# shanedirksen/gnn-plasma-flux

Hardware: AMD Instinct MI355X
Metric: hybrid rollout timesteps/sec (batched ICs) at 1/2/4/8 MI355X (higher is better)
Workload: dtype f32

## Files before the change

gnn-plasma-flux_amd/csrc/chain_bf16.hip:

```cpp
#include "chain_common.h"

namespace hf {
namespace {

using namespace chain;

typedef __bf16 b8 __attribute__((ext_vector_type(8)));
typedef __bf16 b2 __attribute__((ext_vector_type(2)));
typedef float f2 __attribute__((ext_vector_type(2)));
typedef unsigned u4 __attribute__((ext_vector_type(4)));

__device__ __forceinline__ unsigned pk_bf16(float a, float b) {
  return __builtin_bit_cast(unsigned, __builtin_convertvector(f2{a, b}, b2));
}
__device__ __forceinline__ unsigned pk_relu_bf16(float a, float b) { return pk_bf16(relu(a), relu(b)); }
__device__ __forceinline__ f4 mma(const u4 &a, const u4 &b, f4 c) {
  return __builtin_amdgcn_mfma_f32_16x16x32_bf16(__builtin_bit_cast(b8, a), __builtin_bit_cast(b8, b), c, 0, 0, 0);
}

template <int NM, int NV, int ND = 4>
__device__ __forceinline__ void interleave() {
  __builtin_amdgcn_sched_group_barrier(0x100, ND, 0);
#pragma unroll
  for (int i = 0; i < NM; ++i) {
    __builtin_amdgcn_sched_group_barrier(0x008, 1, 0);
    __builtin_amdgcn_sched_group_barrier(0x002, NV, 0);
  }
  __builtin_amdgcn_sched_barrier(0);
}

template <int NW, int UPC, int WMT = 4, bool PF = false, int SLOTS = (UPC == 4 ? 3 : 4), int WG = 1, int DMAU = 0,
          bool XCH = false, bool LDR = false>
struct CoreBF16 {
  static_assert(!XCH || (UPC == 4 && !PF && WMT == 4), "super-window core: 16 KiB chunks, 64-cell waves");
  static constexpr int kNW = NW;
  static constexpr int kWGPerCU = WG;
  static constexpr int kUPC = UPC;
  static constexpr int kSlots = SLOTS;
  static constexpr int kAhead = 2;
  static constexpr int kWinMT = WMT;
  static constexpr int kParkMT = WMT;
  static constexpr int kChunkFloats = 1024 * UPC;
  static constexpr int kKB = kH / 32;
  static constexpr int kStreamOffset = XCH ? kBF16StreamTail : 0;
  static constexpr int kParkFloats = 3 * kParkMT * 64 * 4;
  static constexpr int kSeamF4 = XCH ? 2 * NW * 2 * 4 * 2 : 0;
  static constexpr int kDmaUnit = DMAU;
  using R_t = Ring<kChunkFloats, NW, kSlots, 2, (DMAU >= 0), LDR>;
  static constexpr int pos(int U) { return XCH ? (U + 2) & 3 : U % UPC; }

  template <int MT>
  struct Acts {
    u4 h[MT][kKB];
  };
  template <int MT>
  struct Pair {
    f4 a[MT][2], g[MT][2];
  };

  struct Seam {
    f4 *pubw;
    f4 *rdl;
    f4 *rdr;
    int par;
    static __device__ __forceinline__ int slot(int w, int side) { return (w * 2 + side) * 8; }
    static __device__ __forceinline__ int lane_id() {
      int l;
      asm volatile("v_mbcnt_lo_u32_b32 %0, -1, 0\n\tv_mbcnt_hi_u32_b32 %0, -1, %0" : "=v"(l));
      return l;
    }
  };
  template <int MT>
  static __device__ __forceinline__ void publish(const Seam &sm, const Pair<MT> &P) {
#if defined(HF_DIAG_NOSEAM) || defined(HF_DIAG_NOPUB)
    return;
#endif
    if constexpr (XCH) {
      const int l = Seam::lane_id(), j = l & 15;
      f4 *p = sm.pubw + sm.par * (NW * 16) + ((l >> 4) << 1);
      if (j == 0) {
        p[0] = P.g[1][0];
        p[1] = P.g[1][1];
      }
      if (j == 15) {
        p[8] = P.g[MT - 2][0];
        p[9] = P.g[MT - 2][1];
      }
    }
  }
  static __device__ __forceinline__ void seam_read(const Seam &sm, int t, f4 &L, f4 &R) {
#if defined(HF_DIAG_NOSEAM) || defined(HF_DIAG_NORD)
    L = R = f4{0.f, 0.f, 0.f, 0.f};
    return;
#endif
    const int l = Seam::lane_id(), o = sm.par * (NW * 16) + ((l >> 4) << 1) + t;
    L = sm.rdl[o];
    R = sm.rdr[o];
  }

  struct Feed {
    const float *slot;
    u4 cur[4];
  };
  static __device__ __forceinline__ void load_unit(Feed &F, int u, int lane) {
#pragma unroll
    for (int i = 0; i < 4; ++i) F.cur[i] = __builtin_bit_cast(u4, ldf4(F.slot + ((4 * u + i) * 64 + lane) * 4));
  }
  static __device__ __forceinline__ void begin(R_t &R, Feed &F) {
    F.slot = R.next();
    if constexpr (XCH) R.issue_pending();
    if constexpr (PF) load_unit(F, 0, R.lane);
  }
  template <int U>
  static __device__ __forceinline__ void take(R_t &R, Feed &F, u4 (&w)[4]) {
    if constexpr (PF) {
#pragma unroll
      for (int i = 0; i < 4; ++i) w[i] = F.cur[i];
      if constexpr (U == kDmaUnit) R.issue_pending();
      if constexpr (U == UPC - 1) F.slot = R.next();
      load_unit(F, (U + 1) % UPC, R.lane);
    } else {
#ifdef HF_DIAG_NODS
#pragma unroll
      for (int i = 0; i < 4; ++i) w[i] = u4{(unsigned)R.lane, (unsigned)(4 * U + i), 0x3f803f80u, (unsigned)R.lane};
#else
#pragma unroll
      for (int i = 0; i < 4; ++i) w[i] = __builtin_bit_cast(u4, ldf4(F.slot + ((4 * U + i) * 64 + R.lane) * 4));
#endif
      if constexpr (U == kDmaUnit) R.issue_pending();
      if constexpr (U == UPC - 1) F.slot = R.next();
    }
  }

  static __device__ __forceinline__ float *park_at(float *park, int kb, int mt, int lane) {
    return park + ((kb * kParkMT + mt) * 64 + lane) * 4;
  }

  template <int MT, int KB>
  static __device__ __forceinline__ void unit_mfma(const u4 (&w)[4], const Acts<MT> &X, Pair<MT> &P) {
#pragma unroll
    for (int t = 0; t < 2; ++t)
#pragma unroll
      for (int mt = 0; mt < MT; ++mt) {
        P.a[mt][t] = mma(w[2 * t], X.h[mt][KB], P.a[mt][t]);
        P.g[mt][t] = mma(w[2 * t + 1], X.h[mt][KB], P.g[mt][t]);
      }
  }
  template <int MT, int KB>
  static __device__ __forceinline__ void unit(R_t &R, Feed &F, const Acts<MT> &X, Pair<MT> &P) {
    u4 w[4];
    take<pos(KB)>(R, F, w);
    unit_mfma<MT, KB>(w, X, P);
  }

  template <int MT>
  static __device__ __forceinline__ void init(const float *bias, int q, int g4, Pair<MT> &P) {
#pragma unroll
    for (int t = 0; t < 2; ++t) {
      const f4 b = ldf4(bias + 16 * (2 * q + t) + g4);
#pragma unroll
      for (int mt = 0; mt < MT; ++mt) {
        P.a[mt][t] = b;
        P.g[mt][t] = f4{0.f, 0.f, 0.f, 0.f};
      }
    }
  }

  template <int MT, int K, int PART = 0>
  static __device__ __forceinline__ void piece(Pair<MT> &P, u4 (&nh)[MT], const f4 &L = f4{}, const f4 &R = f4{}) {
    constexpr int t = K >> 1, r0 = 2 * (K & 1);
#ifdef HF_DIAG_NOPIECE
#pragma unroll
    for (int mt = 0; mt < MT; ++mt)
      if (PART == 0 || (PART == 1) == (mt > 0 && mt < MT - 1)) nh[mt][K] = pk_bf16(P.a[mt][t][r0], P.g[mt][t][r0 + 1]);
    return;
#endif
    if constexpr (PART == 0) {
      float z[2][MT];
#pragma unroll
      for (int rr = 0; rr < 2; ++rr) {
        float v[MT], sm[MT];
#pragma unroll
        for (int mt = 0; mt < MT; ++mt) v[mt] = P.g[mt][t][r0 + rr];
        nb_sum<MT>(v, sm);
#pragma unroll
        for (int mt = 0; mt < MT; ++mt) z[rr][mt] = __fadd_rn(P.a[mt][t][r0 + rr], sm[mt]);
      }
#pragma unroll
      for (int mt = 0; mt < MT; ++mt) nh[mt][K] = pk_relu_bf16(z[0][mt], z[1][mt]);
    } else if constexpr (PART == 1) {
#pragma unroll
      for (int mt = 1; mt < MT - 1; ++mt) {
        float z[2];
#pragma unroll
        for (int rr = 0; rr < 2; ++rr) {
          const int r = r0 + rr;
          z[rr] = __fadd_rn(P.a[mt][t][r], __fadd_rn(P.g[mt - 1][t][r], P.g[mt + 1][t][r]));
        }
        nh[mt][K] = pk_relu_bf16(z[0], z[1]);
      }
    } else {
      float z0[2], z1[2];
#pragma unroll
      for (int rr = 0; rr < 2; ++rr) {
        const int r = r0 + rr;
        float sl = __fadd_rn(L[r], P.g[1][t][r]);
        asm("v_add_f32_dpp %0, %1, %2 row_shr:1 row_mask:0xf bank_mask:0xf"
            : "+v"(sl)
            : "v"(P.g[MT - 1][t][r]), "v"(P.g[1][t][r]));
        z0[rr] = __fadd_rn(P.a[0][t][r], sl);
        float sr = __fadd_rn(R[r], P.g[MT - 2][t][r]);
        asm("v_add_f32_dpp %0, %1, %2 row_shl:1 row_mask:0xf bank_mask:0xf"
            : "+v"(sr)
            : "v"(P.g[0][t][r]), "v"(P.g[MT - 2][t][r]));
        z1[rr] = __fadd_rn(P.a[MT - 1][t][r], sr);
      }
      nh[0][K] = pk_relu_bf16(z0[0], z0[1]);
      nh[MT - 1][K] = pk_relu_bf16(z1[0], z1[1]);
    }
  }

  template <int MT>
  static __device__ __forceinline__ void pair_with_prev(R_t &R, Feed &F, const Acts<MT> &X, const float *bias, int q,
                                                        int g4, Pair<MT> &acc, Pair<MT> &prev, float *park,
                                                        int lane, Seam &sm) {
    init<MT>(bias, q, g4, acc);
    u4 nh[MT];
    if constexpr (XCH) {
      unit<MT, 0>(R, F, X, acc);
      piece<MT, 0, 1>(prev, nh);
      piece<MT, 1, 1>(prev, nh);
      interleave<4 * MT, 2>();
      publish<MT>(sm, prev);
      unit<MT, 1>(R, F, X, acc);
      f4 L0, R0;
      seam_read(sm, 0, L0, R0);
      piece<MT, 2, 1>(prev, nh);
      piece<MT, 0, 2>(prev, nh, L0, R0);
      interleave<4 * MT, 2, 2>();
      unit<MT, 2>(R, F, X, acc);
      f4 L1, R1;
      seam_read(sm, 1, L1, R1);
      piece<MT, 3, 1>(prev, nh);
      piece<MT, 1, 2>(prev, nh, L0, R0);
      interleave<4 * MT, 2, 6>();
      unit<MT, 3>(R, F, X, acc);
      piece<MT, 2, 2>(prev, nh, L1, R1);
      piece<MT, 3, 2>(prev, nh, L1, R1);
      sm.par ^= 1;
    } else {
      unit<MT, 0>(R, F, X, acc);
      piece<MT, 0>(prev, nh);
      interleave<4 * MT, 2>();
      unit<MT, 1>(R, F, X, acc);
      piece<MT, 1>(prev, nh);
      interleave<4 * MT, 2>();
      unit<MT, 2>(R, F, X, acc);
      piece<MT, 2>(prev, nh);
      interleave<4 * MT, 2>();
      unit<MT, 3>(R, F, X, acc);
      piece<MT, 3>(prev, nh);
    }
#pragma unroll
    for (int mt = 0; mt < MT; ++mt) *reinterpret_cast<u4 *>(park_at(park, q - 1, mt, lane)) = nh[mt];
    interleave<4 * MT, 2>();
  }

  template <int MT>
  static __device__ __forceinline__ void pair0_after(R_t &R, Feed &F, Acts<MT> &X, const float *bias, int g4,
                                                     Pair<MT> &acc, Pair<MT> &pend, float *park, int lane, Seam &sm) {
    wave_lds_sync();
#pragma unroll
    for (int kb = 0; kb < 3; ++kb)
#pragma unroll
      for (int mt = 0; mt < MT; ++mt) X.h[mt][kb] = __builtin_bit_cast(u4, ldf4(park_at(park, kb, mt, lane)));
    init<MT>(bias, 0, g4, acc);
    u4 nh[MT];
    if constexpr (XCH) {
      unit<MT, 0>(R, F, X, acc);
      piece<MT, 0, 1>(pend, nh);
      piece<MT, 1, 1>(pend, nh);
      piece<MT, 2, 1>(pend, nh);
      interleave<4 * MT, 3>();
      publish<MT>(sm, pend);
      unit<MT, 1>(R, F, X, acc);
      f4 L0, R0, L1, R1;
      seam_read(sm, 0, L0, R0);
      seam_read(sm, 1, L1, R1);
      piece<MT, 3, 1>(pend, nh);
      piece<MT, 0, 2>(pend, nh, L0, R0);
      interleave<4 * MT, 2, 4>();
      unit<MT, 2>(R, F, X, acc);
      piece<MT, 1, 2>(pend, nh, L0, R0);
      piece<MT, 2, 2>(pend, nh, L1, R1);
      piece<MT, 3, 2>(pend, nh, L1, R1);
      interleave<4 * MT, 4>();
      sm.par ^= 1;
    } else {
      unit<MT, 0>(R, F, X, acc);
      piece<MT, 0>(pend, nh);
      piece<MT, 1>(pend, nh);
      interleave<4 * MT, 4>();
      unit<MT, 1>(R, F, X, acc);
      piece<MT, 2>(pend, nh);
      interleave<4 * MT, 2>();
      unit<MT, 2>(R, F, X, acc);
      piece<MT, 3>(pend, nh);
      interleave<4 * MT, 2>();
    }
#pragma unroll
    for (int mt = 0; mt < MT; ++mt) X.h[mt][3] = nh[mt];
    unit<MT, 3>(R, F, X, acc);
    interleave<4 * MT, 0>();
  }

  template <int MT>
  static __device__ __forceinline__ void pair0_first(R_t &R, Feed &F, const Acts<MT> &X, const float *bias, int g4,
                                                     Pair<MT> &acc) {
    init<MT>(bias, 0, g4, acc);
    unit<MT, 0>(R, F, X, acc);
    interleave<4 * MT, 0>();
    unit<MT, 1>(R, F, X, acc);
    interleave<4 * MT, 0>();
    unit<MT, 2>(R, F, X, acc);
    interleave<4 * MT, 0>();
    unit<MT, 3>(R, F, X, acc);
    interleave<4 * MT, 0>();
  }

  template <int MT>
  static __device__ __forceinline__ void pairs_rest(R_t &R, Feed &F, const Acts<MT> &X, const float *bias, int g4,
                                                    Pair<MT> &acc0, Pair<MT> &pend, float *park, int lane, Seam &sm) {
    Pair<MT> acc1, acc2;
    pair_with_prev<MT>(R, F, X, bias, 1, g4, acc1, acc0, park, lane, sm);
    pair_with_prev<MT>(R, F, X, bias, 2, g4, acc2, acc1, park, lane, sm);
    pair_with_prev<MT>(R, F, X, bias, 3, g4, pend, acc2, park, lane, sm);
  }

  template <int MT, int U>
  static __device__ __forceinline__ void ro_mfma(const u4 (&w)[4], const Acts<MT> &X, f4 (&P)[MT], f4 (&Q)[MT]) {
#ifdef HF_DIAG_NOROMFMA
#pragma unroll
    for (int i = 0; i < 4; ++i) asm volatile("" ::"v"(w[i]));
    return;
#endif
#pragma unroll
    for (int i = 0; i < 4; ++i) {
      const int kb = 2 * U + (i >> 1);
#pragma unroll
      for (int mt = 0; mt < MT; ++mt) {
        if (i & 1) Q[mt] = mma(w[i], X.h[mt][kb], Q[mt]);
        else P[mt] = mma(w[i], X.h[mt][kb], P[mt]);
      }
    }
  }
  template <int MT, int U, int T>
  static __device__ __forceinline__ void ro_unit(R_t &R, Feed &F, const Acts<MT> &X, f4 (&P)[MT], f4 (&Q)[MT]) {
    u4 w[4];
    take<T>(R, F, w);
    ro_mfma<MT, U>(w, X, P, Q);
  }

  template <int MT, int RP>
  static __device__ __forceinline__ void ro_piece(const f4 (&P)[MT], const f4 (&Q)[MT], const f4 &w2, float (&pf)[MT],
                                                  float (&pb)[MT]) {
#ifdef HF_DIAG_NOROPIECE
#pragma unroll
    for (int mt = 0; mt < MT; ++mt) pf[mt] += P[mt][2 * RP] + Q[mt][2 * RP + 1];
    return;
#endif
#pragma unroll
    for (int r = 2 * RP; r < 2 * RP + 2; ++r) {
      float pv[MT], qv[MT], pr[MT], qr[MT];
#pragma unroll
      for (int mt = 0; mt < MT; ++mt) {
        pv[mt] = P[mt][r];
        qv[mt] = Q[mt][r];
      }
      right_nb<MT>(pv, pr);
      right_nb<MT>(qv, qr);
#pragma unroll
      for (int mt = 0; mt < MT; ++mt) {
        pf[mt] = fmaf(w2[r], relu(__fadd_rn(pv[mt], qr[mt])), pf[mt]);
        pb[mt] = fmaf(w2[r], relu(__fadd_rn(pr[mt], qv[mt])), pb[mt]);
      }
    }
  }

  template <int MT>
  static __device__ __forceinline__ void init_ro(const Small &S, int ot, int g4, f4 (&P)[MT], f4 (&Q)[MT]) {
    const f4 be = ldf4(S.be + 16 * ot + g4);
#pragma unroll
    for (int mt = 0; mt < MT; ++mt) {
      P[mt] = be;
      Q[mt] = f4{0.f, 0.f, 0.f, 0.f};
    }
  }

  template <int MT, int T0>
  static __device__ __forceinline__ void ro_tile(R_t &R, Feed &F, const Acts<MT> &X, const Small &S, int ot,
                                                 int g4, f4 (&P)[MT], f4 (&Q)[MT], float (&pf)[MT],
                                                 float (&pb)[MT]) {
    f4 Pn[MT], Qn[MT];
    init_ro<MT>(S, ot, g4, Pn, Qn);
    const f4 w2 = ldf4(S.w2 + 16 * (ot - 1) + g4);
    ro_unit<MT, 0, T0>(R, F, X, Pn, Qn);
    ro_piece<MT, 0>(P, Q, w2, pf, pb);
    interleave<4 * MT, 3>();
    ro_unit<MT, 1, T0 + 1>(R, F, X, Pn, Qn);
    ro_piece<MT, 1>(P, Q, w2, pf, pb);
    interleave<4 * MT, 3>();
#pragma unroll
    for (int mt = 0; mt < MT; ++mt) {
      P[mt] = Pn[mt];
      Q[mt] = Qn[mt];
    }
  }

  template <int MT>
  static __device__ __forceinline__ void readout(const ChainW &W, const Small &S, R_t &R, Feed &F, Acts<MT> &X,
                                                 Pair<MT> &pend, float *park, int lane, int g4, float (&ffwd)[MT],
                                                 float (&fbwd)[MT], Seam &sm) {
#ifndef HF_DIAG_NOPARK
    wave_lds_sync();
#pragma unroll
    for (int kb = 0; kb < 3; ++kb)
#pragma unroll
      for (int mt = 0; mt < MT; ++mt) X.h[mt][kb] = __builtin_bit_cast(u4, ldf4(park_at(park, kb, mt, lane)));
#endif
    float pf[MT], pb[MT];
#pragma unroll
    for (int mt = 0; mt < MT; ++mt) pf[mt] = pb[mt] = 0.f;
    f4 P[MT], Q[MT];
    init_ro<MT>(S, 0, g4, P, Q);
    {
      u4 nh[MT];
      if constexpr (XCH) {
        ro_unit<MT, 0, pos(0)>(R, F, X, P, Q);
        piece<MT, 0, 1>(pend, nh);
        piece<MT, 1, 1>(pend, nh);
        piece<MT, 2, 1>(pend, nh);
        piece<MT, 3, 1>(pend, nh);
        interleave<4 * MT, 4>();
        publish<MT>(sm, pend);
        u4 w[4];
        take<pos(1)>(R, F, w);
        f4 L0, R0, L1, R1;
        seam_read(sm, 0, L0, R0);
        seam_read(sm, 1, L1, R1);
        piece<MT, 0, 2>(pend, nh, L0, R0);
        piece<MT, 1, 2>(pend, nh, L0, R0);
        piece<MT, 2, 2>(pend, nh, L1, R1);
        piece<MT, 3, 2>(pend, nh, L1, R1);
        sm.par ^= 1;
#pragma unroll
        for (int mt = 0; mt < MT; ++mt) X.h[mt][3] = nh[mt];
        ro_mfma<MT, 1>(w, X, P, Q);
        interleave<4 * MT, 5>();
      } else {
        ro_unit<MT, 0, 0>(R, F, X, P, Q);
        piece<MT, 0>(pend, nh);
        piece<MT, 1>(pend, nh);
        piece<MT, 2>(pend, nh);
        piece<MT, 3>(pend, nh);
        interleave<4 * MT, 4>();
#pragma unroll
        for (int mt = 0; mt < MT; ++mt) X.h[mt][3] = nh[mt];
        ro_unit<MT, 1, 1>(R, F, X, P, Q);
        interleave<4 * MT, 0>();
      }
    }
    constexpr int kOdd = XCH ? pos(2) : (UPC == 4 ? 2 : 0);
    constexpr int kEven = XCH ? pos(0) : 0;
    for (int ot = 1; ot < kNT - 1; ot += 2) {
      ro_tile<MT, kOdd>(R, F, X, S, ot, g4, P, Q, pf, pb);
      ro_tile<MT, kEven>(R, F, X, S, ot + 1, g4, P, Q, pf, pb);
    }
    ro_tile<MT, kOdd>(R, F, X, S, kNT - 1, g4, P, Q, pf, pb);
    {
      const f4 w2 = ldf4(S.w2 + 16 * (kNT - 1) + g4);
      ro_piece<MT, 0>(P, Q, w2, pf, pb);
      ro_piece<MT, 1>(P, Q, w2, pf, pb);
    }
    readout_finish<MT>(pf, pb, W.b2, ffwd, fbwd);
  }

  template <int MT>
  static __device__ __forceinline__ void input(const Small &S, int lane, const float (&feat)[MT], Acts<MT> &X,
                                               f4 (&h67)[MT][2]) {
#ifdef HF_DIAG_NOINPUT
#pragma unroll
    for (int mt = 0; mt < MT; ++mt) {
      const unsigned v = __float_as_uint(feat[mt]);
#pragma unroll
      for (int kb = 0; kb < kKB; ++kb) X.h[mt][kb] = u4{v, v + kb, v, v};
      h67[mt][0] = h67[mt][1] = f4{feat[mt], feat[mt], feat[mt], feat[mt]};
    }
    return;
#endif
    const int g4 = 4 * (lane >> 4);
    u4 bx[MT];
#pragma unroll
    for (int mt = 0; mt < MT; ++mt) {
      const float hi = __uint_as_float(pk_bf16(feat[mt], 0.f) << 16);
      bx[mt] = u4{pk_bf16(feat[mt], __fsub_rn(feat[mt], hi)), 0u, 0u, 0u};
    }
    const f4 a0 = ldf4(S.win + lane * 4), a1 = ldf4(S.win + 256 + lane * 4);
#pragma unroll
    for (int kb = 0; kb < kKB; ++kb) {
#pragma unroll
      for (int t = 0; t < 2; ++t) {
        const int nt = 2 * kb + t;
        const float w = nt < 4 ? a0[nt & 3] : a1[nt & 3];
        const u4 aw = u4{pk_bf16(w, w), 0u, 0u, 0u};
        const f4 bias = ldf4(S.bin + 16 * nt + g4);
#pragma unroll
        for (int mt = 0; mt < MT; ++mt) {
#ifdef HF_DIAG_NOINMFMA
          asm volatile("" ::"v"(aw), "v"(bx[mt]));
          const f4 h = relu4(bias);
#else
          const f4 h = relu4(mma(aw, bx[mt], bias));
#endif
          X.h[mt][kb][2 * t] = pk_bf16(h[0], h[1]);
          X.h[mt][kb][2 * t + 1] = pk_bf16(h[2], h[3]);
          if (kb == kKB - 1) h67[mt][t] = h;
        }
      }
    }
  }

  template <int MT>
  static __device__ __forceinline__ void gnn_seam(const ChainW &W, const Small &S, R_t &R, Feed &F, float *park,
                                                  Seam &sm, const float (&feat)[MT], float (&ffwd)[MT],
                                                  float (&fbwd)[MT]) {
    const int lane = R.lane;
    const int g4 = 4 * (lane >> 4);
    Acts<MT> X;
    Pair<MT> pend;
    {
      f4 h67[MT][2];
      input<MT>(S, lane, feat, X, h67);
      if (W.layers == 0) {
#ifndef HF_DIAG_NOPARK
#pragma unroll
        for (int kb = 0; kb < 3; ++kb)
#pragma unroll
          for (int mt = 0; mt < MT; ++mt) *reinterpret_cast<u4 *>(park_at(park, kb, mt, lane)) = X.h[mt][kb];
#endif
#pragma unroll
        for (int mt = 0; mt < MT; ++mt) {
          pend.a[mt][0] = h67[mt][0];
          pend.a[mt][1] = h67[mt][1];
          pend.g[mt][0] = pend.g[mt][1] = f4{0.f, 0.f, 0.f, 0.f};
        }
      }
    }
    if (W.layers > 0) {
      Pair<MT> acc0;
      pair0_first<MT>(R, F, X, S.bl, g4, acc0);
      pairs_rest<MT>(R, F, X, S.bl, g4, acc0, pend, park, lane, sm);
    }
    const int nl = __builtin_amdgcn_readfirstlane(W.layers);
    for (int l = 1; l < nl; ++l) {
      const float *bias = S.bl + l * kH;
      Pair<MT> acc0;
      pair0_after<MT>(R, F, X, bias, g4, acc0, pend, park, lane, sm);
      pairs_rest<MT>(R, F, X, bias, g4, acc0, pend, park, lane, sm);
    }
    readout<MT>(W, S, R, F, X, pend, park, lane, g4, ffwd, fbwd, sm);
  }

  template <int MT>
  static __device__ __forceinline__ void gnn(const ChainW &W, const Small &S, R_t &R, Feed &F, float *park,
                                             const float (&feat)[MT], float (&ffwd)[MT], float (&fbwd)[MT]) {
    static_assert(!XCH, "the super-window core runs in chain_flux_sw_kernel");
    Seam sm{};
    gnn_seam<MT>(W, S, R, F, park, sm, feat, ffwd, fbwd);
  }
};

template <class Core>
__global__ __launch_bounds__(64 * Core::kNW, 1) void chain_flux_sw_kernel(ChainW W, const float *__restrict__ nf,
                                                                   const float *__restrict__ state,
                                                                   int64_t ld_state, const float *__restrict__ x,
                                                                   int B, int nx, int nsw,
                                                                   float *__restrict__ fe, float *__restrict__ ff) {
  constexpr int MT = 4, NW = Core::kNW;
  constexpr int kRingFloats = Core::kSlots * Core::kChunkFloats;
  constexpr int kBaseF4 = lds_floats<Core, false>() / 4;
  __shared__ f4 lds4[kBaseF4 + Core::kSeamF4];
  float *lds = reinterpret_cast<float *>(lds4);
  const Small S = stage_small(W, lds + kRingFloats);
  auto R = make_ring<Core>(W, lds);
  const int lane = R.lane, j = lane & 15, g = lane >> 4;
  using Seam = typename Core::Seam;
  Seam sm{lds4 + kBaseF4 + Seam::slot(R.wave, 0), lds4 + kBaseF4 + Seam::slot((R.wave + NW - 1) % NW, 1),
          lds4 + kBaseF4 + Seam::slot((R.wave + 1) % NW, 0), 0};
  __syncthreads();
  R.prime(R.chunks - 1);
  typename Core::Feed F;
  Core::begin(R, F);
  const int L = W.layers;
  const int P = nx + 2 * L + 1;
  const int faces = 63 * NW - 2 * L;
  const int total = B * P;
  auto locate = [&](int s0, int c, int &b, int &p) {
#ifdef HF_DIAG_NOLOC
    b = (s0 < 0 ? 0 : s0) / 1024 % B;
    p = c + L;
    return;
#endif
    const int base = s0 < 0 ? 0 : (s0 >= total ? total - 1 : s0);
    b = base / P;
    int s = s0 + c;
    s = s < 0 ? 0 : (s >= total ? total - 1 : s);
    p = s - b * P;
    while (p >= P) {
      p -= P;
      ++b;
    }
  };
  auto first = [&](int k) { return k * faces - L + 63 * R.wave; };
  auto load_feat = [&](int k, float (&feat)[MT]) {
    const int s0 = __builtin_amdgcn_readfirstlane(first(k));
#pragma unroll
    for (int mt = 0; mt < MT; ++mt) {
      int b, p;
      locate(s0, cell_of<MT>(mt, j), b, p);
      int c = p - L;
      while (c < 0) c += nx;
      while (c >= nx) c -= nx;
#ifdef HF_DIAG_NOFEAT
      feat[mt] = 0.01f * (float)(c + g);
#else
      feat[mt] = nf ? nf[((int64_t)b * nx + c) * kIn + g]
                    : (g < 3 ? state[b * ld_state + (int64_t)g * nx + c] : x[c]);
#endif
    }
  };
  for (int k = blockIdx.x; k < nsw; k += gridDim.x) {
    float feat[MT];
    load_feat(k, feat);
    float f_fwd[MT], f_bwd[MT];
    Core::template gnn_seam<MT>(W, S, R, F, park_of<Core, false>(lds, R.wave), sm, feat, f_fwd, f_bwd);
    const int s0 = __builtin_amdgcn_readfirstlane(first(k));
#pragma unroll
    for (int mt = 0; mt < MT; ++mt) {
      const int c = cell_of<MT>(mt, j), csw = 63 * R.wave + c;
      if (c == 63 || csw < L || csw >= L + faces || s0 + c >= total) continue;
      int b, p;
      locate(s0, c, b, p);
      const int i = p - L;
      if (i < 0 || i >= nx) continue;
#ifdef HF_DIAG_NOFEAT
      if (f_fwd[mt] != 12345.f) continue;
#endif
      if (fe && g == 0) fe[(int64_t)b * 2 * nx + i] = f_fwd[mt];
      if (fe && g == 1) fe[(int64_t)b * 2 * nx + nx + i] = f_bwd[mt];
      if (ff && g == 2) ff[(int64_t)b * nx + i] = face_flux(f_fwd[mt], f_bwd[mt]);
    }
  }
  R.drain();
}

inline int64_t sw_count(int NW, int layers, int64_t B, int nx) {
  const int64_t faces = 63 * NW - 2 * layers, total = B * (nx + 2 * layers + 1);
  return (total + faces - 1) / faces;
}

template <class Core>
hipError_t launch_flux_sw(const ChainW &w, const float *nf, const float *state, int64_t ld_state, const float *x,
                          int B, int nx, float *fe, float *ff, hipStream_t s) {
  const int64_t total = (int64_t)B * (nx + 2 * w.layers + 1);
  if (total >= (int64_t(1) << 31) - 64 * Core::kNW) return hipErrorInvalidValue;
  const int nsw = (int)sw_count(Core::kNW, w.layers, B, nx);
  const int64_t res = resident_groups();
  const int64_t blocks = nsw < res ? nsw : res;
  hipLaunchKernelGGL((chain_flux_sw_kernel<Core>), dim3((unsigned)blocks), dim3(64 * Core::kNW), 0, s, w, nf, state,
                     ld_state, x, B, nx, nsw, fe, ff);
  return hipGetLastError();
}

template <bool LDR = false>
struct CellBF16T {
  using Base = CoreBF16<4, 2, 4, true, 4, 1, -1, false, LDR>;
  static constexpr int kLayerChunks = 8;
  static constexpr bool kLayerBarrier = true;
  static constexpr int kNW = Base::kNW;
  static constexpr int kSlots = Base::kSlots;
  static constexpr int kChunkFloats = Base::kChunkFloats;
  static constexpr int kStreamOffset = 0;
  using R_t = typename Base::R_t;
  using Feed = typename Base::Feed;
  using Acts = typename Base::template Acts<1>;
  using Pair = typename Base::template Pair<1>;
  static __device__ __forceinline__ void begin(R_t &R, Feed &F) { Base::begin(R, F); }

  static __device__ __forceinline__ void gnn_cells(const ChainW &W, const Small &S, R_t &R, Feed &F,
                                                   const float (&feat)[1], float (&ffwd)[1], float (&fbwd)[1],
                                                   CellHalo &X) {
    const int lane = R.lane, g4 = 4 * (lane >> 4);
    Acts A;
    {
      f4 h67[1][2];
      Base::template input<1>(S, lane, feat, A, h67);
    }
    for (int l = 0; l < W.layers; ++l) {
      const float *bias = S.bl + l * kH;
      Pair acc[4];
#pragma unroll
      for (int q = 0; q < 4; ++q) {
        Base::template init<1>(bias, q, g4, acc[q]);
        Base::template unit<1, 0>(R, F, A, acc[q]);
        interleave<4, 0>();
        Base::template unit<1, 1>(R, F, A, acc[q]);
        interleave<4, 0>();
        Base::template unit<1, 2>(R, F, A, acc[q]);
        interleave<4, 0>();
        Base::template unit<1, 3>(R, F, A, acc[q]);
        interleave<4, 0>();
      }
      {
        f4 G[1][kNT];
#pragma unroll
        for (int t = 0; t < kNT; ++t) G[0][t] = acc[t >> 1].g[0][t & 1];
        X.exchange(G);
      }
#pragma unroll
      for (int q = 0; q < 4; ++q)
#pragma unroll
        for (int K = 0; K < 4; ++K) {
          const int tt = K >> 1, t = 2 * q + tt, r0 = 2 * (K & 1);
          float z[2];
#pragma unroll
          for (int rr = 0; rr < 2; ++rr) {
            const int r = r0 + rr;
            const float v = acc[q].g[0][tt][r];
            const float gl = dpp_over<kRowShr1>(X.l[t][r], v), gr = dpp_over<kRowShl1>(X.r[t][r], v);
            z[rr] = __fadd_rn(acc[q].a[0][tt][r], __fadd_rn(gl, gr));
          }
          A.h[0][q][K] = pk_relu_bf16(z[0], z[1]);
        }
    }
    const int j = lane & 15, g = lane >> 4;
    f4 P[kNT][1], Q[kNT][1];
#pragma unroll
    for (int ot = 0; ot < kNT; ++ot) {
      Base::template init_ro<1>(S, ot, g4, P[ot], Q[ot]);
      Base::template ro_unit<1, 0, 0>(R, F, A, P[ot], Q[ot]);
      interleave<4, 0>();
      Base::template ro_unit<1, 1, 1>(R, F, A, P[ot], Q[ot]);
      interleave<4, 0>();
      if (j == 0) {
        X.xq[((X.wave * kNT + ot) * 2 + 0) * 4 + g] = P[ot][0];
        X.xq[((X.wave * kNT + ot) * 2 + 1) * 4 + g] = Q[ot][0];
      }
    }
    lds_barrier();
    float pf = 0.f, pb = 0.f;
#pragma unroll
    for (int ot = 0; ot < kNT; ++ot) {
      const f4 prh = X.xq[((X.rw * kNT + ot) * 2 + 0) * 4 + g];
      const f4 qrh = X.xq[((X.rw * kNT + ot) * 2 + 1) * 4 + g];
      const f4 w2 = ldf4(S.w2 + 16 * ot + g4);
#pragma unroll
      for (int r = 0; r < 4; ++r) {
        const float pv = P[ot][0][r], qv = Q[ot][0][r];
        const float pr = dpp_over<kRowShl1>(prh[r], pv), qr = dpp_over<kRowShl1>(qrh[r], qv);
        pf = fmaf(w2[r], relu(__fadd_rn(pv, qr)), pf);
        pb = fmaf(w2[r], relu(__fadd_rn(pr, qv)), pb);
      }
    }
    float pf1[1] = {pf}, pb1[1] = {pb};
    readout_finish<1>(pf1, pb1, W.b2, ffwd, fbwd);
  }
};
using CellBF16Ld = CellBF16T<true>;

}

using SwCoreBF16 = CoreBF16<8, 4, 4, false, 3, 1, 0, true>;

hipError_t launch_chain_flux_bf16(const ChainW &w, const float *nf, const float *state, int64_t ld_state,
                                  const float *x, int B, int nx, float *fe, float *ff, hipStream_t s) {
  if (B <= 0) return hipSuccess;
  if (chain_rollout_prefers_cells(w, B, nx)) {
    switch (nx) {
      case 32: return chain::flux_cells_launch<CellBF16Ld, 2>(w, nf, state, ld_state, x, B, fe, ff, s);
      case 48: return chain::flux_cells_launch<CellBF16Ld, 3>(w, nf, state, ld_state, x, B, fe, ff, s);
      case 64: return chain::flux_cells_launch<CellBF16Ld, 4>(w, nf, state, ld_state, x, B, fe, ff, s);
      default: break;
    }
  }
  if (nx == 16 || nx == 32 || nx == 48 || nx == 64)
    return chain::launch_flux_core<CoreBF16<8, 4>>(w, nf, state, ld_state, x, B, nx, fe, ff, s);
  return launch_flux_sw<SwCoreBF16>(w, nf, state, ld_state, x, B, nx, fe, ff, s);
}

FluxWork chain_flux_work(const ChainW &w, int64_t B, int nx) {
  FluxWork fw;
  if (w.prec != kPrecBF16 || B <= 0 || nx == 16 || nx == 32 || nx == 48 || nx == 64 ||
      chain_rollout_prefers_cells(w, (int)B, nx))
    return fw;
  fw.units = sw_count(SwCoreBF16::kNW, w.layers, B, nx);

  fw.per_round = resident_groups();
  return fw;
}

hipError_t launch_chain_rollout_bf16(const ChainW &w, const float *state0, float *state_final, const float *x,
                                     const double *pc, int B, int nx, int T, float c, float dt, float *traj,
                                     float *flux_traj, float *metrics, const RolloutExtras &ex, hipStream_t s) {
  if (ex.mse == nullptr && ex.metrics_cl == nullptr && chain_rollout_prefers_cells(w, B, nx)) {
    switch (nx) {
      case 32: return chain::cells_launch<CellBF16Ld, 2>(w, state0, state_final, x, pc, B, T, c, dt, traj, flux_traj, metrics, ex.poisson, s);
      case 48: return chain::cells_launch<CellBF16Ld, 3>(w, state0, state_final, x, pc, B, T, c, dt, traj, flux_traj, metrics, ex.poisson, s);
      case 64: return chain::cells_launch<CellBF16Ld, 4>(w, state0, state_final, x, pc, B, T, c, dt, traj, flux_traj, metrics, ex.poisson, s);
      default: break;
    }
  }
  return chain::launch_rollout_core<CoreBF16<4, 2, 4, true, 4, 1, -1>>(w, state0, state_final, x, pc, B, nx, T, c, dt, traj,
                                                             flux_traj, metrics, ex, s);
}

}
```

Baseline: 6.688 million.

## Replace seam-sum exchange with bf16 activation halo cells between super-window waves

Before, neighbouring waves exchanged f32 partial message sums across a seam. The new code instead overlaps waves by one cell (62-cell stride instead of 63). Each wave writes its edge activations, already packed to bf16, straight into the neighbour's park buffer, and publishes a small halo slot for the last sub-block. The edge pieces are now computed with DPP zero-fill like the inner ones, and the piece/seam scheduling is restructured around the halo exchange. The intent is to cut the exchanged data and the dependent seam reads in the inner pair loop. The cost is one redundant cell per wave, which slightly lowers faces per super-window, plus changed synchronization assumptions around park writes.

Result: no change. 6.699 million, median of 4 (+0.2%).

```diff
diff --git a/gnn-plasma-flux_amd/csrc/chain_bf16.hip b/gnn-plasma-flux_amd/csrc/chain_bf16.hip
--- a/gnn-plasma-flux_amd/csrc/chain_bf16.hip
+++ b/gnn-plasma-flux_amd/csrc/chain_bf16.hip
@@ -20,7 +20,7 @@
 
 template <int NM, int NV, int ND = 4>
 __device__ __forceinline__ void interleave() {
-  __builtin_amdgcn_sched_group_barrier(0x100, ND, 0);
+  if constexpr (ND > 0) __builtin_amdgcn_sched_group_barrier(0x100, ND, 0);
 #pragma unroll
   for (int i = 0; i < NM; ++i) {
     __builtin_amdgcn_sched_group_barrier(0x008, 1, 0);
@@ -44,7 +44,7 @@
   static constexpr int kKB = kH / 32;
   static constexpr int kStreamOffset = XCH ? kBF16StreamTail : 0;
   static constexpr int kParkFloats = 3 * kParkMT * 64 * 4;
-  static constexpr int kSeamF4 = XCH ? 2 * NW * 2 * 4 * 2 : 0;
+  static constexpr int kHaloF4 = XCH ? 2 * NW * 2 * 4 : 0;
   static constexpr int kDmaUnit = DMAU;
   using R_t = Ring<kChunkFloats, NW, kSlots, 2, (DMAU >= 0), LDR>;
   static constexpr int pos(int U) { return XCH ? (U + 2) & 3 : U % UPC; }
@@ -58,12 +58,13 @@
     f4 a[MT][2], g[MT][2];
   };
 
-  struct Seam {
-    f4 *pubw;
-    f4 *rdl;
-    f4 *rdr;
+  using u4_t = u4;
+  struct Halo {
+    float *lpark, *rpark;
+    u4 *pub;
+    u4 *rdl, *rdr;
     int par;
-    static __device__ __forceinline__ int slot(int w, int side) { return (w * 2 + side) * 8; }
+    bool has_l, has_r;
     static __device__ __forceinline__ int lane_id() {
       int l;
       asm volatile("v_mbcnt_lo_u32_b32 %0, -1, 0\n\tv_mbcnt_hi_u32_b32 %0, -1, %0" : "=v"(l));
@@ -71,31 +72,50 @@
     }
   };
   template <int MT>
-  static __device__ __forceinline__ void publish(const Seam &sm, const Pair<MT> &P) {
-#if defined(HF_DIAG_NOSEAM) || defined(HF_DIAG_NOPUB)
-    return;
-#endif
-    if constexpr (XCH) {
-      const int l = Seam::lane_id(), j = l & 15;
-      f4 *p = sm.pubw + sm.par * (NW * 16) + ((l >> 4) << 1);
-      if (j == 0) {
-        p[0] = P.g[1][0];
-        p[1] = P.g[1][1];
-      }
-      if (j == 15) {
-        p[8] = P.g[MT - 2][0];
-        p[9] = P.g[MT - 2][1];
-      }
-    }
-  }
-  static __device__ __forceinline__ void seam_read(const Seam &sm, int t, f4 &L, f4 &R) {
-#if defined(HF_DIAG_NOSEAM) || defined(HF_DIAG_NORD)
-    L = R = f4{0.f, 0.f, 0.f, 0.f};
-    return;
-#endif
-    const int l = Seam::lane_id(), o = sm.par * (NW * 16) + ((l >> 4) << 1) + t;
-    L = sm.rdl[o];
-    R = sm.rdr[o];
+  static __device__ __forceinline__ void park_store(float *park, int kb, int lane, const u4 (&nh)[MT]) {
+#pragma unroll
+    for (int mt = XCH ? 1 : 0; mt < (XCH ? MT - 1 : MT); ++mt)
+      *reinterpret_cast<u4 *>(park_at(park, kb, mt, lane)) = nh[mt];
+  }
+  template <int MT>
+  static __device__ __forceinline__ void park_edges(const Halo &H, float *park, int kb, const u4 (&nh)[MT]) {
+    static_assert(MT >= 4, "distinct edge and halo tiles");
+    const int l = Halo::lane_id(), j = l & 15;
+    if (H.has_l && j == 0) {
+      *reinterpret_cast<u4 *>(park_at(H.lpark, kb, MT - 1, l + 15)) = nh[1];
+      asm volatile("");
+    } else {
+      *reinterpret_cast<u4 *>(park_at(park, kb, 0, l)) = nh[0];
+    }
+    if (H.has_r && j == 15) {
+      *reinterpret_cast<u4 *>(park_at(H.rpark, kb, 0, l - 15)) = nh[MT - 2];
+      asm volatile("");
+    } else {
+      *reinterpret_cast<u4 *>(park_at(park, kb, MT - 1, l)) = nh[MT - 1];
+    }
+  }
+  template <int MT>
+  static __device__ __forceinline__ void publish(const Halo &H, const u4 (&nh)[MT]) {
+    const int l = Halo::lane_id(), j = l & 15;
+    u4 *p = H.pub + H.par * (NW * 8) + (l >> 4);
+    if (H.has_l && j == 0) p[0] = nh[1];
+    if (H.has_r && j == 15) p[4] = nh[MT - 2];
+  }
+  static __device__ __forceinline__ void halo_read(const Halo &H, u4 &L, u4 &R) {
+    const int o = H.par * (NW * 8) + (Halo::lane_id() >> 4);
+    L = H.rdl[o];
+    R = H.rdr[o];
+  }
+  template <int MT>
+  static __device__ __forceinline__ void halo_take(Halo &H, u4 (&nh)[MT], const u4 &L, const u4 &R) {
+    const int j = Halo::lane_id() & 15;
+    const bool hl = H.has_l && j == 0, hr = H.has_r && j == 15;
+#pragma unroll
+    for (int e = 0; e < 4; ++e) {
+      nh[0][e] = hl ? L[e] : nh[0][e];
+      nh[MT - 1][e] = hr ? R[e] : nh[MT - 1][e];
+    }
+    H.par ^= 1;
   }
 
   struct Feed {
@@ -167,111 +187,75 @@
   }
 
   template <int MT, int K, int PART = 0>
-  static __device__ __forceinline__ void piece(Pair<MT> &P, u4 (&nh)[MT], const f4 &L = f4{}, const f4 &R = f4{}) {
+  static __device__ __forceinline__ void piece(Pair<MT> &P, u4 (&nh)[MT]) {
+    static_assert(PART == 0 || XCH, "tile subsets: the super-window core");
     constexpr int t = K >> 1, r0 = 2 * (K & 1);
 #ifdef HF_DIAG_NOPIECE
 #pragma unroll
-    for (int mt = 0; mt < MT; ++mt)
-      if (PART == 0 || (PART == 1) == (mt > 0 && mt < MT - 1)) nh[mt][K] = pk_bf16(P.a[mt][t][r0], P.g[mt][t][r0 + 1]);
+    for (int mt = 0; mt < MT; ++mt) nh[mt][K] = pk_bf16(P.a[mt][t][r0], P.g[mt][t][r0 + 1]);
     return;
 #endif
-    if constexpr (PART == 0) {
-      float z[2][MT];
-#pragma unroll
-      for (int rr = 0; rr < 2; ++rr) {
-        float v[MT], sm[MT];
-#pragma unroll
-        for (int mt = 0; mt < MT; ++mt) v[mt] = P.g[mt][t][r0 + rr];
-        nb_sum<MT>(v, sm);
-#pragma unroll
-        for (int mt = 0; mt < MT; ++mt) z[rr][mt] = __fadd_rn(P.a[mt][t][r0 + rr], sm[mt]);
-      }
-#pragma unroll
-      for (int mt = 0; mt < MT; ++mt) nh[mt][K] = pk_relu_bf16(z[0][mt], z[1][mt]);
-    } else if constexpr (PART == 1) {
-#pragma unroll
-      for (int mt = 1; mt < MT - 1; ++mt) {
+    if constexpr (XCH) {
+#pragma unroll
+      for (int mt = 0; mt < MT; ++mt) {
+        if (PART != 0 && (PART == 1) != (mt > 0 && mt < MT - 1)) continue;
         float z[2];
 #pragma unroll
         for (int rr = 0; rr < 2; ++rr) {
           const int r = r0 + rr;
-          z[rr] = __fadd_rn(P.a[mt][t][r], __fadd_rn(P.g[mt - 1][t][r], P.g[mt + 1][t][r]));
+          float s;
+          if (mt == 0) s = __fadd_rn(dpp_zero<kRowRor1>(P.g[MT - 1][t][r]), P.g[1][t][r]);
+          else if (mt == MT - 1) s = __fadd_rn(dpp_zero<kRowRor15>(P.g[0][t][r]), P.g[MT - 2][t][r]);
+          else s = __fadd_rn(P.g[mt - 1][t][r], P.g[mt + 1][t][r]);
+          z[rr] = __fadd_rn(P.a[mt][t][r], s);
         }
         nh[mt][K] = pk_relu_bf16(z[0], z[1]);
       }
-    } else {
-      float z0[2], z1[2];
-#pragma unroll
-      for (int rr = 0; rr < 2; ++rr) {
-        const int r = r0 + rr;
-        float sl = __fadd_rn(L[r], P.g[1][t][r]);
-        asm("v_add_f32_dpp %0, %1, %2 row_shr:1 row_mask:0xf bank_mask:0xf"
-            : "+v"(sl)
-            : "v"(P.g[MT - 1][t][r]), "v"(P.g[1][t][r]));
-        z0[rr] = __fadd_rn(P.a[0][t][r], sl);
-        float sr = __fadd_rn(R[r], P.g[MT - 2][t][r]);
-        asm("v_add_f32_dpp %0, %1, %2 row_shl:1 row_mask:0xf bank_mask:0xf"
-            : "+v"(sr)
-            : "v"(P.g[0][t][r]), "v"(P.g[MT - 2][t][r]));
-        z1[rr] = __fadd_rn(P.a[MT - 1][t][r], sr);
-      }
-      nh[0][K] = pk_relu_bf16(z0[0], z0[1]);
-      nh[MT - 1][K] = pk_relu_bf16(z1[0], z1[1]);
-    }
+      return;
+    }
+    float z[2][MT];
+#pragma unroll
+    for (int rr = 0; rr < 2; ++rr) {
+      float v[MT], sm[MT];
+#pragma unroll
+      for (int mt = 0; mt < MT; ++mt) v[mt] = P.g[mt][t][r0 + rr];
+      nb_sum<MT>(v, sm);
+#pragma unroll
+      for (int mt = 0; mt < MT; ++mt) z[rr][mt] = __fadd_rn(P.a[mt][t][r0 + rr], sm[mt]);
+    }
+#pragma unroll
+    for (int mt = 0; mt < MT; ++mt) nh[mt][K] = pk_relu_bf16(z[0][mt], z[1][mt]);
   }
 
   template <int MT>
   static __device__ __forceinline__ void pair_with_prev(R_t &R, Feed &F, const Acts<MT> &X, const float *bias, int q,
                                                         int g4, Pair<MT> &acc, Pair<MT> &prev, float *park,
-                                                        int lane, Seam &sm) {
+                                                        int lane, const Halo &H) {
     init<MT>(bias, q, g4, acc);
     u4 nh[MT];
-    if constexpr (XCH) {
-      unit<MT, 0>(R, F, X, acc);
-      piece<MT, 0, 1>(prev, nh);
-      piece<MT, 1, 1>(prev, nh);
-      interleave<4 * MT, 2>();
-      publish<MT>(sm, prev);
-      unit<MT, 1>(R, F, X, acc);
-      f4 L0, R0;
-      seam_read(sm, 0, L0, R0);
-      piece<MT, 2, 1>(prev, nh);
-      piece<MT, 0, 2>(prev, nh, L0, R0);
-      interleave<4 * MT, 2, 2>();
-      unit<MT, 2>(R, F, X, acc);
-      f4 L1, R1;
-      seam_read(sm, 1, L1, R1);
-      piece<MT, 3, 1>(prev, nh);
-      piece<MT, 1, 2>(prev, nh, L0, R0);
-      interleave<4 * MT, 2, 6>();
-      unit<MT, 3>(R, F, X, acc);
-      piece<MT, 2, 2>(prev, nh, L1, R1);
-      piece<MT, 3, 2>(prev, nh, L1, R1);
-      sm.par ^= 1;
-    } else {
-      unit<MT, 0>(R, F, X, acc);
-      piece<MT, 0>(prev, nh);
-      interleave<4 * MT, 2>();
-      unit<MT, 1>(R, F, X, acc);
-      piece<MT, 1>(prev, nh);
-      interleave<4 * MT, 2>();
-      unit<MT, 2>(R, F, X, acc);
-      piece<MT, 2>(prev, nh);
-      interleave<4 * MT, 2>();
-      unit<MT, 3>(R, F, X, acc);
-      piece<MT, 3>(prev, nh);
-    }
-#pragma unroll
-    for (int mt = 0; mt < MT; ++mt) *reinterpret_cast<u4 *>(park_at(park, q - 1, mt, lane)) = nh[mt];
+    unit<MT, 0>(R, F, X, acc);
+    piece<MT, 0>(prev, nh);
     interleave<4 * MT, 2>();
+    unit<MT, 1>(R, F, X, acc);
+    piece<MT, 1>(prev, nh);
+    interleave<4 * MT, 2>();
+    unit<MT, 2>(R, F, X, acc);
+    piece<MT, 2>(prev, nh);
+    interleave<4 * MT, 2>();
+    unit<MT, 3>(R, F, X, acc);
+    piece<MT, 3>(prev, nh);
+    park_store<MT>(park, q - 1, lane, nh);
+    if constexpr (XCH) asm volatile("" ::"v"(nh[0]), "v"(nh[MT - 1]));
+    interleave<4 * MT, 2>();
+    if constexpr (XCH) park_edges<MT>(H, park, q - 1, nh);
   }
 
   template <int MT>
   static __device__ __forceinline__ void pair0_after(R_t &R, Feed &F, Acts<MT> &X, const float *bias, int g4,
-                                                     Pair<MT> &acc, Pair<MT> &pend, float *park, int lane, Seam &sm) {
+                                                     Pair<MT> &acc, Pair<MT> &pend, float *park, int lane, Halo &H) {
     wave_lds_sync();
 #pragma unroll
-    for (int kb = 0; kb < 3; ++kb)
+    for (int kb = 0; kb < (XCH ? 2 : 3); ++kb)
 #pragma unroll
       for (int mt = 0; mt < MT; ++mt) X.h[mt][kb] = __builtin_bit_cast(u4, ldf4(park_at(park, kb, mt, lane)));
     init<MT>(bias, 0, g4, acc);
@@ -281,21 +265,22 @@
       piece<MT, 0, 1>(pend, nh);
       piece<MT, 1, 1>(pend, nh);
       piece<MT, 2, 1>(pend, nh);
+      piece<MT, 3, 1>(pend, nh);
+      interleave<4 * MT, 4>();
+      publish<MT>(H, nh);
+      unit<MT, 1>(R, F, X, acc);
+#pragma unroll
+      for (int mt = 0; mt < MT; ++mt) X.h[mt][2] = __builtin_bit_cast(u4, ldf4(park_at(park, 2, mt, lane)));
+      u4 hl, hr;
+      halo_read(H, hl, hr);
+      piece<MT, 0, 2>(pend, nh);
+      piece<MT, 1, 2>(pend, nh);
+      interleave<4 * MT, 2, MT + 2>();
+      unit<MT, 2>(R, F, X, acc);
+      piece<MT, 2, 2>(pend, nh);
+      piece<MT, 3, 2>(pend, nh);
+      halo_take<MT>(H, nh, hl, hr);
       interleave<4 * MT, 3>();
-      publish<MT>(sm, pend);
-      unit<MT, 1>(R, F, X, acc);
-      f4 L0, R0, L1, R1;
-      seam_read(sm, 0, L0, R0);
-      seam_read(sm, 1, L1, R1);
-      piece<MT, 3, 1>(pend, nh);
-      piece<MT, 0, 2>(pend, nh, L0, R0);
-      interleave<4 * MT, 2, 4>();
-      unit<MT, 2>(R, F, X, acc);
-      piece<MT, 1, 2>(pend, nh, L0, R0);
-      piece<MT, 2, 2>(pend, nh, L1, R1);
-      piece<MT, 3, 2>(pend, nh, L1, R1);
-      interleave<4 * MT, 4>();
-      sm.par ^= 1;
     } else {
       unit<MT, 0>(R, F, X, acc);
       piece<MT, 0>(pend, nh);
@@ -330,11 +315,12 @@
 
   template <int MT>
   static __device__ __forceinline__ void pairs_rest(R_t &R, Feed &F, const Acts<MT> &X, const float *bias, int g4,
-                                                    Pair<MT> &acc0, Pair<MT> &pend, float *park, int lane, Seam &sm) {
+                                                    Pair<MT> &acc0, Pair<MT> &pend, float *park, int lane,
+                                                    const Halo &H) {
     Pair<MT> acc1, acc2;
-    pair_with_prev<MT>(R, F, X, bias, 1, g4, acc1, acc0, park, lane, sm);
-    pair_with_prev<MT>(R, F, X, bias, 2, g4, acc2, acc1, park, lane, sm);
-    pair_with_prev<MT>(R, F, X, bias, 3, g4, pend, acc2, park, lane, sm);
+    pair_with_prev<MT>(R, F, X, bias, 1, g4, acc1, acc0, park, lane, H);
+    pair_with_prev<MT>(R, F, X, bias, 2, g4, acc2, acc1, park, lane, H);
+    pair_with_prev<MT>(R, F, X, bias, 3, g4, pend, acc2, park, lane, H);
   }
 
   template <int MT, int U>
@@ -420,11 +406,11 @@
   template <int MT>
   static __device__ __forceinline__ void readout(const ChainW &W, const Small &S, R_t &R, Feed &F, Acts<MT> &X,
                                                  Pair<MT> &pend, float *park, int lane, int g4, float (&ffwd)[MT],
-                                                 float (&fbwd)[MT], Seam &sm) {
+                                                 float (&fbwd)[MT], Halo &H) {
 #ifndef HF_DIAG_NOPARK
     wave_lds_sync();
 #pragma unroll
-    for (int kb = 0; kb < 3; ++kb)
+    for (int kb = 0; kb < (XCH ? 2 : 3); ++kb)
 #pragma unroll
       for (int mt = 0; mt < MT; ++mt) X.h[mt][kb] = __builtin_bit_cast(u4, ldf4(park_at(park, kb, mt, lane)));
 #endif
@@ -437,26 +423,23 @@
       u4 nh[MT];
       if constexpr (XCH) {
         ro_unit<MT, 0, pos(0)>(R, F, X, P, Q);
-        piece<MT, 0, 1>(pend, nh);
-        piece<MT, 1, 1>(pend, nh);
-        piece<MT, 2, 1>(pend, nh);
-        piece<MT, 3, 1>(pend, nh);
-        interleave<4 * MT, 4>();
-        publish<MT>(sm, pend);
+        piece<MT, 0>(pend, nh);
+        piece<MT, 1>(pend, nh);
+        piece<MT, 2>(pend, nh);
+        piece<MT, 3>(pend, nh);
+        interleave<4 * MT, 8>();
+        publish<MT>(H, nh);
         u4 w[4];
         take<pos(1)>(R, F, w);
-        f4 L0, R0, L1, R1;
-        seam_read(sm, 0, L0, R0);
-        seam_read(sm, 1, L1, R1);
-        piece<MT, 0, 2>(pend, nh, L0, R0);
-        piece<MT, 1, 2>(pend, nh, L0, R0);
-        piece<MT, 2, 2>(pend, nh, L1, R1);
-        piece<MT, 3, 2>(pend, nh, L1, R1);
-        sm.par ^= 1;
+#pragma unroll
+        for (int mt = 0; mt < MT; ++mt) X.h[mt][2] = __builtin_bit_cast(u4, ldf4(park_at(park, 2, mt, lane)));
+        u4 hl, hr;
+        halo_read(H, hl, hr);
+        halo_take<MT>(H, nh, hl, hr);
 #pragma unroll
         for (int mt = 0; mt < MT; ++mt) X.h[mt][3] = nh[mt];
         ro_mfma<MT, 1>(w, X, P, Q);
-        interleave<4 * MT, 5>();
+        interleave<4 * MT, 1, MT + 2>();
       } else {
         ro_unit<MT, 0, 0>(R, F, X, P, Q);
         piece<MT, 0>(pend, nh);
@@ -531,8 +514,8 @@
   }
 
   template <int MT>
-  static __device__ __forceinline__ void gnn_seam(const ChainW &W, const Small &S, R_t &R, Feed &F, float *park,
-                                                  Seam &sm, const float (&feat)[MT], float (&ffwd)[MT],
+  static __device__ __forceinline__ void gnn_halo(const ChainW &W, const Small &S, R_t &R, Feed &F, float *park,
+                                                  Halo &H, const float (&feat)[MT], float (&ffwd)[MT],
                                                   float (&fbwd)[MT]) {
     const int lane = R.lane;
     const int g4 = 4 * (lane >> 4);
@@ -559,24 +542,24 @@
     if (W.layers > 0) {
       Pair<MT> acc0;
       pair0_first<MT>(R, F, X, S.bl, g4, acc0);
-      pairs_rest<MT>(R, F, X, S.bl, g4, acc0, pend, park, lane, sm);
+      pairs_rest<MT>(R, F, X, S.bl, g4, acc0, pend, park, lane, H);
     }
     const int nl = __builtin_amdgcn_readfirstlane(W.layers);
     for (int l = 1; l < nl; ++l) {
       const float *bias = S.bl + l * kH;
       Pair<MT> acc0;
-      pair0_after<MT>(R, F, X, bias, g4, acc0, pend, park, lane, sm);
-      pairs_rest<MT>(R, F, X, bias, g4, acc0, pend, park, lane, sm);
-    }
-    readout<MT>(W, S, R, F, X, pend, park, lane, g4, ffwd, fbwd, sm);
+      pair0_after<MT>(R, F, X, bias, g4, acc0, pend, park, lane, H);
+      pairs_rest<MT>(R, F, X, bias, g4, acc0, pend, park, lane, H);
+    }
+    readout<MT>(W, S, R, F, X, pend, park, lane, g4, ffwd, fbwd, H);
   }
 
   template <int MT>
   static __device__ __forceinline__ void gnn(const ChainW &W, const Small &S, R_t &R, Feed &F, float *park,
                                              const float (&feat)[MT], float (&ffwd)[MT], float (&fbwd)[MT]) {
     static_assert(!XCH, "the super-window core runs in chain_flux_sw_kernel");
-    Seam sm{};
-    gnn_seam<MT>(W, S, R, F, park, sm, feat, ffwd, fbwd);
+    Halo H{};
+    gnn_halo<MT>(W, S, R, F, park, H, feat, ffwd, fbwd);
   }
 };
 
@@ -589,21 +572,25 @@
   constexpr int MT = 4, NW = Core::kNW;
   constexpr int kRingFloats = Core::kSlots * Core::kChunkFloats;
   constexpr int kBaseF4 = lds_floats<Core, false>() / 4;
-  __shared__ f4 lds4[kBaseF4 + Core::kSeamF4];
+  __shared__ f4 lds4[kBaseF4 + Core::kHaloF4];
   float *lds = reinterpret_cast<float *>(lds4);
   const Small S = stage_small(W, lds + kRingFloats);
   auto R = make_ring<Core>(W, lds);
-  const int lane = R.lane, j = lane & 15, g = lane >> 4;
-  using Seam = typename Core::Seam;
-  Seam sm{lds4 + kBaseF4 + Seam::slot(R.wave, 0), lds4 + kBaseF4 + Seam::slot((R.wave + NW - 1) % NW, 1),
-          lds4 + kBaseF4 + Seam::slot((R.wave + 1) % NW, 0), 0};
+  const int j = R.lane & 15, g = R.lane >> 4;
+  typename Core::Halo H;
+  H.has_l = R.wave > 0, H.has_r = R.wave + 1 < NW;
+  const int wl = H.has_l ? R.wave - 1 : R.wave, wr = H.has_r ? R.wave + 1 : R.wave;
+  H.lpark = park_of<Core, false>(lds, wl), H.rpark = park_of<Core, false>(lds, wr);
+  typename Core::u4_t *hs = reinterpret_cast<typename Core::u4_t *>(lds4 + kBaseF4);
+  H.pub = hs + R.wave * 8, H.rdl = hs + wl * 8 + 4, H.rdr = hs + wr * 8;
+  H.par = 0;
   __syncthreads();
   R.prime(R.chunks - 1);
   typename Core::Feed F;
   Core::begin(R, F);
   const int L = W.layers;
   const int P = nx + 2 * L + 1;
-  const int faces = 63 * NW - 2 * L;
+  const int faces = 62 * NW + 1 - 2 * L;
   const int total = B * P;
   auto locate = [&](int s0, int c, int &b, int &p) {
 #ifdef HF_DIAG_NOLOC
@@ -621,7 +608,7 @@
       ++b;
     }
   };
-  auto first = [&](int k) { return k * faces - L + 63 * R.wave; };
+  auto first = [&](int k) { return k * faces - L + 62 * R.wave; };
   auto load_feat = [&](int k, float (&feat)[MT]) {
     const int s0 = __builtin_amdgcn_readfirstlane(first(k));
 #pragma unroll
@@ -643,12 +630,12 @@
     float feat[MT];
     load_feat(k, feat);
     float f_fwd[MT], f_bwd[MT];
-    Core::template gnn_seam<MT>(W, S, R, F, park_of<Core, false>(lds, R.wave), sm, feat, f_fwd, f_bwd);
+    Core::template gnn_halo<MT>(W, S, R, F, park_of<Core, false>(lds, R.wave), H, feat, f_fwd, f_bwd);
     const int s0 = __builtin_amdgcn_readfirstlane(first(k));
 #pragma unroll
     for (int mt = 0; mt < MT; ++mt) {
-      const int c = cell_of<MT>(mt, j), csw = 63 * R.wave + c;
-      if (c == 63 || csw < L || csw >= L + faces || s0 + c >= total) continue;
+      const int c = cell_of<MT>(mt, j), csw = 62 * R.wave + c;
+      if (c == 63 || (c == 62 && H.has_r) || csw < L || csw >= L + faces || s0 + c >= total) continue;
       int b, p;
       locate(s0, c, b, p);
       const int i = p - L;
@@ -665,7 +652,7 @@
 }
 
 inline int64_t sw_count(int NW, int layers, int64_t B, int nx) {
-  const int64_t faces = 63 * NW - 2 * layers, total = B * (nx + 2 * layers + 1);
+  const int64_t faces = 62 * NW + 1 - 2 * layers, total = B * (nx + 2 * layers + 1);
   return (total + faces - 1) / faces;
 }
 
```
